# dmytroleonenko/gym-narde

Hardware: AMD Instinct MI355X
Metric: env steps/sec at batch=65536, 1 MI355X (+ legal-move bit-exact vs CPU) (higher is better)
Workload: dtype u32

## Files before the change

__graft_entry__.py:

```python
import os
import subprocess
import sys

ROOT = os.path.dirname(os.path.abspath(__file__))
PKG_DIR = os.path.join(ROOT, "gym-narde_amd")
CSRC = os.path.join(PKG_DIR, "csrc")
LIB = os.path.join(PKG_DIR, "gym_narde", "libnarde.so")
HOSTCHECK = os.path.join(ROOT, "tests", "hostcheck")

HIPCC = os.environ.get("HIPCC", "/opt/rocm/bin/hipcc")
HIP_FLAGS = ["-O3", "-std=c++17", "--offload-arch=gfx950", "-fPIC", "-shared", "-Wall"]


def _paths():
    for p in (PKG_DIR, os.path.join(ROOT, "oracle")):
        if p not in sys.path:
            sys.path.insert(0, p)


def _run(cmd):
    print("+", " ".join(cmd), flush=True)
    subprocess.check_call(cmd)


def build():
    srcs = [os.path.join(CSRC, "narde.hip"), os.path.join(CSRC, "dqn_learner.hip")]
    _run([HIPCC, *HIP_FLAGS, "-o", LIB, *srcs])
    _run(["make", "-s", "-C", os.path.join(ROOT, "oracle")])
    os.makedirs(os.path.join(HOSTCHECK, "build"), exist_ok=True)
    _run([HIPCC, "-O2", "-std=c++17", "-fPIC", "-shared", "-x", "c++", "-D__HIP_PLATFORM_AMD__",
          "-I/opt/rocm/include", "-o", os.path.join(HOSTCHECK, "build", "libhostcheck.so"),
          os.path.join(HOSTCHECK, "hostcheck.cpp")])
    _run([HIPCC, "-O2", "-std=c++17", "-fPIC", "-shared", "-x", "c++", "-D__HIP_PLATFORM_AMD__",
          "-I/opt/rocm/include", "-o", os.path.join(HOSTCHECK, "build", "libhostcheck_afterstates.so"),
          os.path.join(HOSTCHECK, "hostcheck_afterstates.cpp")])
    _run([HIPCC, "-O2", "-std=c++17", "-fPIC", "-shared", "-x", "c++", "-D__HIP_PLATFORM_AMD__",
          "-I/opt/rocm/include", "-o", os.path.join(HOSTCHECK, "build", "libhostcheck_turn_afterstates.so"),
          os.path.join(HOSTCHECK, "hostcheck_turn_afterstates.cpp")])
    _run([HIPCC, "-O2", "-std=c++17", "-fPIC", "-shared", "-x", "c++", "-D__HIP_PLATFORM_AMD__",
          "-I/opt/rocm/include", "-o", os.path.join(HOSTCHECK, "build", "libhostcheck_value.so"),
          os.path.join(HOSTCHECK, "hostcheck_value.cpp")])
    _run([HIPCC, "-O2", "-std=c++17", "-fPIC", "-shared", "-x", "c++", "-D__HIP_PLATFORM_AMD__",
          "-I/opt/rocm/include", "-o", os.path.join(HOSTCHECK, "build", "libhostcheck_td.so"),
          os.path.join(HOSTCHECK, "hostcheck_td.cpp")])
    _run([HIPCC, "-O2", "-std=c++17", "-fPIC", "-shared", "-x", "c++", "-D__HIP_PLATFORM_AMD__",
          "-I/opt/rocm/include", "-o", os.path.join(HOSTCHECK, "build", "libhostcheck_lookahead.so"),
          os.path.join(HOSTCHECK, "hostcheck_lookahead.cpp")])
    _run([HIPCC, "-O2", "-std=c++17", "-fPIC", "-shared", "-x", "c++", "-D__HIP_PLATFORM_AMD__",
          "-I/opt/rocm/include", "-o", os.path.join(HOSTCHECK, "build", "libhostcheck_turn_lookahead.so"),
          os.path.join(HOSTCHECK, "hostcheck_turn_lookahead.cpp")])
    _run([HIPCC, "-O2", "-std=c++17", "-fPIC", "-shared", "-x", "c++", "-D__HIP_PLATFORM_AMD__",
          "-I/opt/rocm/include", "-o", os.path.join(HOSTCHECK, "build", "libhostcheck_value_rollout.so"),
          os.path.join(HOSTCHECK, "hostcheck_value_rollout.cpp")])
    _run([HIPCC, "-O2", "-std=c++17", "-fPIC", "-shared", "-x", "c++", "-D__HIP_PLATFORM_AMD__",
          "-I/opt/rocm/include", "-o", os.path.join(HOSTCHECK, "build", "libhostcheck_turn_value_rollout.so"),
          os.path.join(HOSTCHECK, "hostcheck_turn_value_rollout.cpp")])
    _paths()
    import gym_narde
    import gym_narde.envs
    import gym_narde.vector
    from gym_narde import _lib

    _lib.load()


def smoke():
    _paths()
    import numpy as np
    import torch

    import oracle as O
    from gym_narde.envs.narde import Narde
    from gym_narde.vector import VecNardeEnv

    assert torch.cuda.is_available(), "smoke() needs a GPU"
    n, plies, seed = 2048, 64, 20251015
    env = VecNardeEnv(n, device="cuda:0", seed=seed, env_id_offset=5, max_episode_steps=1000)
    ref = O.SelfPlay(n, seed=seed, env0=5)
    ref.reset(0)
    rec = ref.run(plies)
    for p in range(plies):
        obs, rew, term, trunc, info = env.step()
        torch.cuda.synchronize()
        assert np.array_equal(obs.cpu().numpy(), rec["obs"][p].astype(np.int32)), f"obs ply {p}"
        assert np.array_equal(rew.cpu().numpy(), rec["reward"][p].astype(np.int32)), f"reward ply {p}"
        assert np.array_equal(term.cpu().numpy(), rec["terminated"][p]), f"terminated ply {p}"
        assert np.array_equal(info["actions"].cpu().numpy(), rec["action"][p]), f"actions ply {p}"
        assert np.array_equal(info["legal"].cpu().numpy().view(np.uint64), rec["legal"][p]), f"legal ply {p}"
    st = env.get_state()
    assert np.array_equal(st["board"].cpu().numpy(), ref.board)
    g = Narde()
    assert g.get_valid_moves([5, 3], 1) == [(23, 18)]
    assert g.get_valid_moves([6, 6], 1) == [(23, 17), (23, 17)]
    env.close()
    _smoke_turn_value_rollout(torch, VecNardeEnv, seed)
    print(f"smoke ok: {n} envs x {plies} plies bit-exact vs oracle; FULL4 value rollout = the composed loop")


def _smoke_turn_value_rollout(torch, VecNardeEnv, seed):
    from gym_narde.value_net import ValueMLP

    B, plies = 64, 3
    torch.manual_seed(seed)
    net = ValueMLP(80, "sigmoid", "sigmoid").to("cuda:0")
    one, loop = (VecNardeEnv(B, device="cuda:0", seed=seed, rules="full4") for _ in range(2))
    bufs = one.turn_value_rollout(plies, net)
    for k in range(plies):
        dice = loop.dice()
        aft, values = loop.scored_turn_afterstates(net, dice=dice)
# ... 21 lines not shown
```

gym-narde_amd/csrc/full4_wave.h:

```cpp
#pragma once

namespace {

__device__ __forceinline__ uint32_t rl(uint32_t v, int l) {
  return (uint32_t)__builtin_amdgcn_readlane((int)v, l);
}
__device__ void coop_run(const Side& s, uint32_t low, int a, int b, int hl, uint32_t m0, uint32_t m1,
                         int need, bool bf, int mode, int lane, uint32_t out[3]) {
  out[0] = out[1] = out[2] = 0u;
  uint64_t owners = __ballot((m0 | m1) != 0u);
  const int which = lane >> 5, p = lane & 31;
  while (owners) {
    const int ow = (int)__builtin_ctzll(owners);
    owners &= owners - 1ull;
    Side c;
    c.own.w[0] = rl(s.own.w[0], ow); c.own.w[1] = rl(s.own.w[1], ow); c.own.w[2] = rl(s.own.w[2], ow);
    c.O = rl(s.O, ow); c.S1o = rl(s.S1o, ow); c.P = rl(s.P, ow);
    c.off_own = rl(s.off_own, ow);
    c.opp.w[0] = c.opp.w[1] = c.opp.w[2] = 0u;
    c.S1p = 0u; c.off_opp = 0u; c.ft_own = 0u; c.ft_opp = 0u; c.black = 0u; c.elapsed = 0u; c.t = 0u;
    const uint32_t lw = rl(low, ow), om0 = rl(m0, ow), om1 = rl(m1, ow);
    const int pa = (int)rl((uint32_t)a, ow), pb = (int)rl((uint32_t)b, ow);
    const int thl = (int)rl((uint32_t)hl, ow), tneed = (int)rl((uint32_t)need, ow);
    const bool tbf = rl(bf ? 1u : 0u, ow) != 0u;
// ... 219 lines not shown
    c.O = rl(s.O, ow); c.S1o = rl(s.S1o, ow); c.P = rl(s.P, ow);
    c.off_own = rl(s.off_own, ow);
    c.opp.w[0] = c.opp.w[1] = c.opp.w[2] = 0u;
    c.S1p = 0u; c.off_opp = 0u; c.ft_own = 0u; c.ft_opp = 0u; c.black = 0u; c.elapsed = 0u; c.t = 0u;
    const uint32_t ofw = rl(fw, ow), om = rl(m0, ow), ow0 = rl(w0, ow);
    const int od = (int)rl((uint32_t)d, ow), ohl = (int)rl((uint32_t)hl, ow);
    const int nsrc = __builtin_popcount(om);
    const int r = lane >> 3, k = lane & 7;
    const bool hs = r < nsrc;
    const int s0 = select_bit(om, hs ? r : 0);
    Side ca = c;
    apply_die_if(ca, s0, od, hs);
    const int hla = ohl - ((hs && s0 == 23) ? 1 : 0);
    uint32_t L1 = die_candidates_sl(ca.O, ca.P, od);
    L1 &= ~block_reject_w(ca.O, ca.S1o, ofw, L1, od);
    L1 &= hla <= 0 ? ~HEAD : ~0u;
    L1 = hs ? L1 : 0u;
    const int cnt = __builtin_popcount(L1);
    if (nsrc > 8 || __ballot(k == 0 && cnt > 8) != 0ull) continue;
    const bool hp = k < cnt;
    const int s1 = select_bit(L1, hp ? k : 0);
    Side cp = ca;
    apply_die_if(cp, s1, od, hp);
    const int hlp = hla - ((hp && s1 == 23) ? 1 : 0);
    int dep = f4_probe_w<2>(cp, ofw, od, hlp);
    const bool miss = hp && dep == 1;
    if (__ballot(miss) != 0ull) {
      if (miss) dep = f4_depth_w<2>(cp, ofw, od, hlp);
    }
    const uint64_t B0 = __ballot(k == 0 && cnt > 0), B1 = __ballot(hp && dep >= 1), B2 = __ballot(hp && dep >= 2);
    const bool src = lane < 24 && ((om >> lane) & 1u);
    const int rt = __builtin_popcount(om & ((1u << (lane & 31)) - 1u));
    const int sh = src ? 8 * rt : 0;
    const uint32_t a0 = (uint32_t)__ballot(src && ((B0 >> sh) & 1ull) != 0ull);
    const uint32_t a1 = (uint32_t)__ballot(src && ((B1 >> sh) & 0xFFull) != 0ull);
    const uint32_t a2 = (uint32_t)__ballot(src && ((B2 >> sh) & 0xFFull) != 0ull);
    const int M = a2 ? 4 : (a1 ? 3 : (a0 ? 2 : 1));
    const uint32_t Cs = a2 ? a2 : (a1 ? a1 : (a0 ? a0 : om));
    const int p0 = select_bit(Cs, (int)mulhi_u32(ow0, (uint32_t)__builtin_popcount(Cs)));
    const int r0p = __builtin_popcount(om & ((1u << p0) - 1u));
    const uint32_t Lp = rl(L1, 8 * r0p);
    const uint32_t G = (uint32_t)(((M >= 4 ? B2 : B1) >> (8 * r0p)) & 0xFFull);
    const bool inl = lane < 24 && ((Lp >> lane) & 1u);
    const int e = __builtin_popcount(Lp & ((1u << (lane & 31)) - 1u));
    const uint32_t cv = (uint32_t)__ballot(inl && ((G >> e) & 1u));
    r0[0] = lane == ow ? a0 : r0[0];
    r0[1] = lane == ow ? a1 : r0[1];
    r0[2] = lane == ow ? a2 : r0[2];
    c1 = lane == ow ? cv : c1;
    ok = lane == ow ? true : ok;
  }
}

__device__ __forceinline__ void ply_bound_turn_c0(Side& s, int dh, int dl, uint32_t bs, uint32_t fw,
                                                  const uint32_t w[4], bool flip_always, TurnOut& o, int lane,
                                                  const TurnC0& c) {
  uint32_t Lh = c.Lh, Ll = c.Ll, Ch = c.Ch, Cl = c.Cl;
  int M = c.M;
  const int hl0 = c.hl0;
  const bool dbl = dh == dl;
  const bool b2 = bs != 0u && !dbl, bd = bs != 0u && dbl;
  if (__ballot(b2) != 0ull) {
    if (b2) turn_c0_pair_bound_w(s, dh, dl, bs, fw, Lh, Ll, Ch, Cl, M);
  }
  bool srch = false, pairs = false;
  uint32_t c1p = 0u;
  if (__ballot(bd) != 0ull) {
    const uint32_t Lb = Lh & ~block_reject_w(s.O, s.S1o, bd ? fw : 0u, Lh, dh);
    const bool fast = bd && f4_safe_bound(s, dh, hl0, bs) >= 4;
    srch = bd && !fast && Lb != 0u;
    uint32_t r0[3];
    coop_pair_w(s, fw, dh, hl0, srch ? Lb : 0u, w[0], lane, r0, c1p, pairs);
    if (__ballot(srch && !pairs) != 0ull) {
      uint32_t rd[3];
      coop_depth_w(s, fw, dh, hl0, (srch && !pairs) ? Lb : 0u, 3, lane, rd);
      if (srch && !pairs) { r0[0] = rd[0]; r0[1] = rd[1]; r0[2] = rd[2]; }
    }
    const int Ms = r0[2] ? 4 : (r0[1] ? 3 : (r0[0] ? 2 : 1));
    const uint32_t Cs = r0[2] ? r0[2] : (r0[1] ? r0[1] : (r0[0] ? r0[0] : Lb));
    Ch = bd ? (fast ? Lb : (Lb ? Cs : 0u)) : Ch;
    M = bd ? (fast ? 4 : (Lb ? Ms : 0)) : M;
  }
  o.legal = (uint64_t)Ch | ((uint64_t)Cl << 24) | ((uint64_t)dh << 48) | ((uint64_t)dl << 52) |
            ((uint64_t)M << 56);
  const int nh = __builtin_popcount(Ch), n = nh + __builtin_popcount(Cl);
  const int idx = (int)mulhi_u32(w[0], (uint32_t)n);
  const bool hi = idx < nh;
  const int d0 = hi ? dh : dl;
  const int p0 = select_bit(hi ? Ch : Cl, hi ? idx : idx - nh);
  const bool go = M >= 1;
  apply_die_if(s, p0, d0, go);
  uint32_t pl0 = go ? (0xFFFF0000u | ((uint32_t)d0 << 8) | (uint32_t)p0) : 0xFFFFFFFFu, pl1 = 0xFFFFFFFFu;
  int hl = hl0 - ((go && p0 == 23) ? 1 : 0);
  const int d1 = dbl ? dh : (d0 == dh ? dl : dh);
  const bool anyb = __ballot(bs != 0u) != 0ull;
#pragma unroll
  for (int k = 1; k < 4; ++k) {
    const int dk = k == 1 ? d1 : dh;
    const bool act = k < M;
    uint32_t Lk = die_candidates_sl(s.O, s.P, dk);
    if (anyb) {
      const bool filt = bd || (k == 1 && b2);
      Lk &= ~block_reject_w(s.O, s.S1o, filt ? fw : 0u, Lk, dk);
    }
    Lk &= hl <= 0 ? ~HEAD : ~0u;
    const int need = M - k - 1;
    const bool byp = k == 1 && pairs && need > 0;
    Lk = (srch && act && byp) ? c1p : Lk;
    const bool chk = srch && act && need > 0 && !byp;
    if (__ballot(chk) != 0ull) {
      uint32_t rk[3];
      coop_depth_w(s, fw, dk, hl, chk ? Lk : 0u, need, lane, rk);
      Lk = chk ? (need >= 2 ? rk[1] : rk[0]) : Lk;
    }
    const uint32_t wk = k == 1 ? w[1] : (k == 2 ? w[2] : w[3]);
    const int p = select_bit(Lk, (int)mulhi_u32(wk, (uint32_t)__builtin_popcount(Lk)));
    apply_die_if(s, p, dk, act);
    const uint32_t v = ((uint32_t)dk << 8) | (uint32_t)p;
    if (k == 1) pl0 = act ? ((pl0 & 0xFFFFu) | (v << 16)) : pl0;
    if (k == 2) pl1 = act ? ((pl1 & 0xFFFF0000u) | v) : pl1;
    if (k == 3) pl1 = act ? ((pl1 & 0xFFFFu) | (v << 16)) : pl1;
    hl -= (act && p == 23) ? 1 : 0;
  }
  o.played = (uint64_t)pl0 | ((uint64_t)pl1 << 32);
  o.max_dice = M;
  o.term = s.off_own == 15u;
  o.reward = o.term ? (s.off_opp > 0u ? 1 : 2) : 0;
  if (flip_always) side_flip(s);
  else side_flip_if(s, !o.term);
}

__device__ __forceinline__ void ply_bound_turn(Side& s, int dh, int dl, uint32_t bs, uint32_t fw, const uint32_t w[4],
                                               bool flip_always, TurnOut& o, int lane) {
  TurnC0 c;
  turn_c0_free(s, dh, dl, c.Lh, c.Ll, c.Ch, c.Cl, c.M, c.hl0);
  ply_bound_turn_c0(s, dh, dl, bs, fw, w, flip_always, o, lane, c);
}

}
```

gym-narde_amd/csrc/kernels_rollout.h:

```cpp
#pragma once

namespace {

struct Outs {
  int32_t* __restrict__ obs;
  int32_t* __restrict__ reward;
  uint8_t* __restrict__ term;
  uint8_t* __restrict__ trunc;
  uint64_t* __restrict__ legal;
  int16_t* __restrict__ act_out;
  uint64_t* __restrict__ played;
  int64_t* __restrict__ totals;
};

struct StepArgs {
  Planes pl;
  int n;
  Rng g;
  int max_steps;
  int autoreset;
  const int16_t* __restrict__ actions;
  const int8_t* __restrict__ play;
  const uint8_t* __restrict__ dice;
  Outs out;
// ... 97 lines not shown

__device__ __forceinline__ void store_outs(const Outs& out, size_t ix, const Side& s,
                                           const TurnOut& o, int term, int trunc, int4* lds,
                                           bool wave_full) {
  (void)wave_full;
  store_common(out, ix, s, o.reward, term, trunc, lds, false);
  if (out.legal) st_nt(out.legal + ix, o.legal);
  if (out.played) st_nt(out.played + ix, o.played);
}

#define OBS_LDS_DECL                                   \
  __shared__ int4 obs_lds[kBlock * 6];                 \
  int4* const wave_lds = obs_lds + (threadIdx.x & ~63) * 6;

__device__ __forceinline__ void ply_draw_cached(const Rng& g, uint32_t t, uint32_t i, uint32_t R[4], bool first,
                                                uint32_t r[4]) {
  if (first || (t & 1u) == 0u) ply_block(t, g.env0 + i, g.k0, g.k1, R);
  ply_words_of(R, t, g.dice_mode, r);
}

__device__ __forceinline__ void ply(Side& s, int4& st, const Rng& g, uint32_t i,
                                    const int16_t* actions, const uint8_t* dice, int max_steps,
                                    bool autoreset, StepOut& o, int& term, int& trunc, uint32_t R[4],
                                    bool first) {
  uint32_t r[4];
  ply_draw_cached(g, s.t, i, R, first, r);
  int d0 = 0, d1 = 0, c1 = 0, c2 = 0;
  if (dice) { d0 = dice[2 * i]; d1 = dice[2 * i + 1]; }
  if (actions) { c1 = actions[2 * i]; c2 = actions[2 * i + 1]; }
  if (!dice && !actions && autoreset) env_ply_policy_sl(s, st, r, g.dice_mode, max_steps, o, term, trunc);
  else env_ply(s, st, r, dice != nullptr, d0, d1, g.dice_mode, actions == nullptr, c1, c2, max_steps,
               autoreset, o, term, trunc);
}

__device__ __forceinline__ void ply_draw_wave(const Rng& g, uint32_t t, uint32_t i, uint32_t R[4], int p, int par,
                                              uint32_t r[4]) {
  if (par >= 0) {
    if (p == 0 || ((par + p) & 1) == 0) ply_block(t, g.env0 + i, g.k0, g.k1, R);
  } else if (p == 0 || (t & 1u) == 0u) {
    ply_block(t, g.env0 + i, g.k0, g.k1, R);
  }
  ply_words_of(R, t, g.dice_mode, r);
}

__device__ __forceinline__ int wave_parity(bool valid, uint32_t t) {
  const uint64_t odd = __ballot(valid && (t & 1u)), vm = __ballot(valid);
  return odd == 0ull ? 0 : (odd == vm ? 1 : -1);
}

template <bool kFilt>
__device__ __forceinline__ void ply_free_turn(Side& s, int dh, int dl, uint32_t bs, uint32_t fw, const uint32_t w[4],
                                              bool flip_always, TurnOut& o, const TurnC0& c) {
  uint32_t Lh = c.Lh, Ll = c.Ll, Ch = c.Ch, Cl = c.Cl;
  int M = c.M;
  const bool b2 = kFilt && bs != 0u;
  if (kFilt && b2) turn_c0_pair_bound_w(s, dh, dl, bs, fw, Lh, Ll, Ch, Cl, M);
  turn_moves_sl(s, dh, dl, Ch, Cl, M, c.hl0, w, b2, fw, flip_always, o);
}

__device__ __forceinline__ void ply_full_turn(Side& s, int4& st, int dh, int dl, uint32_t bs, uint32_t fw,
                                              const TurnC0& c, const uint32_t w[4], uint32_t rb, int max_steps,
                                              bool autoreset, TurnOut& o, int& term, int& trunc) {
  const uint32_t mover_black = s.black;
  if (__ballot(bs != 0u && dh == dl) == 0ull) {
    if (__ballot(bs != 0u) == 0ull) ply_free_turn<false>(s, dh, dl, bs, fw, w, autoreset, o, c);
    else ply_free_turn<true>(s, dh, dl, bs, fw, w, autoreset, o, c);
  } else {
    ply_bound_turn_c0(s, dh, dl, bs, fw, w, autoreset, o, (int)(threadIdx.x & 63), c);
  }
  if (autoreset) ply_close_sl_b(s, st, o.term, o.reward, mover_black, rb, max_steps, term, trunc);
  else ply_close(s, st, o.term, o.reward, mover_black, 0u, max_steps, false, term, trunc);
}

__device__ __forceinline__ void ply_full_dice(Side& s, int4& st, int dh, int dl, const uint32_t w[4], uint32_t rb,
                                              int max_steps, bool autoreset, TurnOut& o, int& term, int& trunc) {
  const uint32_t low = block_lowmask(s.P);
  uint32_t fw;
  const uint32_t bs = turn_block_set_sl(s.O, s.S1o, s.P, low, dh, dl, fw);
  TurnC0 c;
  turn_c0_free(s, dh, dl, c.Lh, c.Ll, c.Ch, c.Cl, c.M, c.hl0);
  ply_full_turn(s, st, dh, dl, bs, fw, c, w, rb, max_steps, autoreset, o, term, trunc);
}

__device__ __forceinline__ uint32_t ply_dice_word(const uint32_t r[4], int dice_mode, uint32_t w[4]) {
  int d0, d1;
  dice_from(r[0], dice_mode, d0, d1);
  const int dh = d0 > d1 ? d0 : d1, dl = d0 > d1 ? d1 : d0;
  turn_words(r, w);
  return (uint32_t)dh | ((uint32_t)dl << 4) | (reset_black(r[3]) << 8);
}

__device__ __forceinline__ void ply_full_words(Side& s, int4& st, const uint32_t r[4], int dice_mode,
                                               int max_steps, bool autoreset, TurnOut& o, int& term,
                                               int& trunc) {
  uint32_t w[4];
  const uint32_t dw = ply_dice_word(r, dice_mode, w);
  ply_full_dice(s, st, (int)(dw & 15u), (int)((dw >> 4) & 15u), w, autoreset ? dw >> 8 : 0u, max_steps, autoreset,
                o, term, trunc);
}

__device__ __forceinline__ void ply_policy_full(Side& s, int4& st, const Rng& g, uint32_t i, int max_steps,
                                                bool autoreset, TurnOut& o, int& term, int& trunc,
                                                uint32_t R[4], int p, int par) {
  uint32_t r[4];
  ply_draw_wave(g, s.t, i, R, p, par, r);
  ply_full_words(s, st, r, g.dice_mode, max_steps, autoreset, o, term, trunc);
}

__device__ __forceinline__ void ply(Side& s, int4& st, const Rng& g, uint32_t i, bool valid,
                                    const int8_t* play, const uint8_t* dice, int max_steps,
                                    bool autoreset, TurnOut& o, int& term, int& trunc, uint32_t R[4],
                                    bool first) {
  if (!play && !dice) {
    ply_policy_full(s, st, g, i, max_steps, autoreset, o, term, trunc, R, 0, 0);
    return;
  }
  uint32_t r[4];
  ply_draw_cached(g, s.t, i, R, first, r);
  int d0 = 1, d1 = 2;
  if (dice && valid) { d0 = dice[2 * i]; d1 = dice[2 * i + 1]; }
  const uint64_t pw = (play && valid) ? reinterpret_cast<const uint64_t*>(play)[i] : ~0ull;
  const int lane = (int)(threadIdx.x & 63);
  env_ply_full_with(s, st, r, g.env0 + i, g.k0, g.k1, dice != nullptr, d0, d1, g.dice_mode,
                    play != nullptr, pw, max_steps, autoreset, o, term, trunc,
                    [&](Side& s2, int a, int b, bool pl, uint64_t pw2, const uint32_t* w2, TurnOut& o2) {
                      coop_turn_full(s2, a, b, pl, pw2, w2, o2, lane);
                    });
}

__device__ __forceinline__ void add_stats(int4* __restrict__ stats, int i, const int4& st) {
  if (st.x) {
    int4 cur = stats[i];
    cur.x += st.x; cur.y += st.y; cur.z += st.z;
// ... 402 lines not shown
```

gym-narde_amd/csrc/narde_rules.h:

```cpp
#pragma once
#include <hip/hip_runtime.h>
#include <math.h>
#include <stdint.h>

#define NARDE_FN __host__ __device__ __forceinline__

namespace narde {

constexpr uint32_t MASK24 = 0xFFFFFFu;
constexpr int OFF = 24;

struct Nib {
  uint32_t w[3];
};

NARDE_FN uint32_t funnel16(uint32_t hi, uint32_t lo) { return (lo >> 16) | (hi << 16); }

NARDE_FN uint32_t nib_word(const Nib& b, int p) {
  const uint32_t w0 = b.w[0], w1 = b.w[1], w2 = b.w[2];
  const int k = p >> 3;
  return (k == 0 ? w0 : 0u) | (k == 1 ? w1 : 0u) | (k == 2 ? w2 : 0u);
}
NARDE_FN uint32_t nib_get(const Nib& b, int p) { return (nib_word(b, p) >> (4 * (p & 7))) & 15u; }
NARDE_FN void nib_add(Nib& b, int p, uint32_t delta ) {
// ... 1136 lines not shown
  return L & (e1 | e2 | e3);
}

NARDE_FN bool f4_bearoff_fixed_sl(const Side& s, int rem) {
  uint32_t x = s.own.w[0] & 0xFFFFFFu;
  x = (x & 0x0F0F0Fu) + ((x >> 4) & 0x0F0F0Fu);
  const uint32_t home = ((x * 0x010101u) >> 16) & 0xFFu;
  return ((s.O >> 6) == 0u) | ((int)(15u - s.off_own - home) >= rem);
}

NARDE_FN int f4_open_moves_sl(const Side& s, int d, int hl, int T) {
  const uint32_t O = s.O, fr = ~s.P & MASK24;
  const uint32_t r0 = (1u << d) - 1u;
  const uint32_t r1 = ((r0 & fr) << d) & MASK24;
  const uint32_t r2 = ((r1 & fr) << d) & MASK24;
  const uint32_t r3 = ((r2 & fr) << d) & MASK24;
  const uint32_t R = (r0 | r1 | r2 | r3) & O;
  const uint32_t h1 = ((0x3Fu & fr) << d) & MASK24;
  const uint32_t h2 = ((h1 & fr) << d) & MASK24;
  const uint32_t h3 = ((h2 & fr) << d) & MASK24;
  const uint32_t X = O & ~0x3Fu;
  const int head = (int)nib_get(s.own, 23);
  const bool reach = (X & ~(h1 | h2 | h3)) == 0u && !((X & HEAD) && head > hl);
  uint32_t ge4;
  const uint32_t ge3 = nib_ge3_ge4(s.own, ge4);
  const uint32_t Rb = R & ~HEAD;
  const int B = __builtin_popcount(Rb) + __builtin_popcount(Rb & ~s.S1o) + __builtin_popcount(Rb & ge3) +
                __builtin_popcount(Rb & ge4) + ((R & HEAD) ? head : 0);
  const int t = T + (reach ? B : 0);
  return t < 4 ? t : 4;
}

NARDE_FN void turn_c0_free(const Side& s, int dh, int dl, uint32_t& Lh, uint32_t& Ll, uint32_t& Ch, uint32_t& Cl,
                           int& M, int& hl0) {
  const bool dbl = dh == dl;
  Lh = die_candidates_sl(s.O, s.P, dh);
  Ll = die_candidates_sl(s.O, s.P, dl) & msk(!dbl);
  const uint32_t kh = f4_keep_pair_bf_sl(s.O, s.S1o, s.P, dh, dl, Lh);
  const uint32_t kl = f4_keep_pair_bf_sl(s.O, s.S1o, s.P, dl, dh, Ll);
  hl0 = (dbl && s.ft_own && (dh == 3 || dh == 4 || dh == 6)) ? 2 : 1;
  const int T0 = f4_exact_moves(s, dh, hl0);
  const int Mo = f4_open_moves_sl(s, dh, hl0, T0);
  const int Mx = f4_bearoff_fixed_sl(s, 4) ? T0 : Mo;
  const bool pair = (kh | kl) != 0u;
  const bool two = !dbl && pair;
  Ch = (kh & msk(two)) | (Lh & msk(!two));
  Cl = (kl & msk(two)) | (Ll & msk(!dbl && !pair && Lh == 0u));
  const int M2 = two ? 2 : ((Lh | Ll) != 0u ? 1 : 0);
  M = dbl ? (Lh != 0u ? Mx : 0) : M2;
}

struct TurnC0 {
  uint32_t Lh, Ll, Ch, Cl;
  int M, hl0;
};

NARDE_FN void side_flip_if(Side& s, bool flip) {
  Side f = s;
  side_flip(f);
  s.own.w[0] = flip ? f.own.w[0] : s.own.w[0];
  s.own.w[1] = flip ? f.own.w[1] : s.own.w[1];
  s.own.w[2] = flip ? f.own.w[2] : s.own.w[2];
  s.opp.w[0] = flip ? f.opp.w[0] : s.opp.w[0];
  s.opp.w[1] = flip ? f.opp.w[1] : s.opp.w[1];
  s.opp.w[2] = flip ? f.opp.w[2] : s.opp.w[2];
  s.O = flip ? f.O : s.O;
  s.P = flip ? f.P : s.P;
  s.S1o = flip ? f.S1o : s.S1o;
  s.S1p = flip ? f.S1p : s.S1p;
  s.off_own = flip ? f.off_own : s.off_own;
  s.off_opp = flip ? f.off_opp : s.off_opp;
  s.ft_own = flip ? f.ft_own : s.ft_own;
  s.ft_opp = flip ? f.ft_opp : s.ft_opp;
  s.black = flip ? f.black : s.black;
}

NARDE_FN uint32_t block_reject_w(uint32_t O, uint32_t S1, uint32_t fw, uint32_t C, int d);
NARDE_FN void turn_moves_sl(Side& s, int dh, int dl, uint32_t Ch, uint32_t Cl, int M, int hl, const uint32_t w[4],
                            bool filt, uint32_t fw, bool flip_always, TurnOut& o) {
  const bool dbl = dh == dl;
  o.legal = (uint64_t)Ch | ((uint64_t)Cl << 24) | ((uint64_t)dh << 48) | ((uint64_t)dl << 52) |
            ((uint64_t)M << 56);
  const int nh = __builtin_popcount(Ch), n = nh + __builtin_popcount(Cl);
  const int idx = (int)mulhi_u32(w[0], (uint32_t)n);
  const bool hi = idx < nh;
  const int d0 = hi ? dh : dl;
  const int p0 = select_bit(hi ? Ch : Cl, hi ? idx : idx - nh);
  const bool go = M >= 1;
  apply_die_if(s, p0, d0, go);
  uint32_t pl0 = go ? (0xFFFF0000u | ((uint32_t)d0 << 8) | (uint32_t)p0) : 0xFFFFFFFFu, pl1 = 0xFFFFFFFFu;
  hl -= (go && p0 == 23) ? 1 : 0;
  const int d1 = dbl ? dh : (d0 == dh ? dl : dh);
#pragma unroll
  for (int k = 1; k < 4; ++k) {
    const int dk = k == 1 ? d1 : dh;
    const bool act = k < M;
    uint32_t Lk = die_candidates_sl(s.O, s.P, dk);
    if (k == 1 && filt) Lk &= ~block_reject_w(s.O, s.S1o, fw, Lk, dk);
    Lk &= hl <= 0 ? ~HEAD : ~0u;
    const uint32_t wk = k == 1 ? w[1] : (k == 2 ? w[2] : w[3]);
    const int p = select_bit(Lk, (int)mulhi_u32(wk, (uint32_t)__builtin_popcount(Lk)));
    apply_die_if(s, p, dk, act);
    const uint32_t v = ((uint32_t)dk << 8) | (uint32_t)p;
    if (k == 1) pl0 = act ? ((pl0 & 0xFFFFu) | (v << 16)) : pl0;
    if (k == 2) pl1 = act ? ((pl1 & 0xFFFF0000u) | v) : pl1;
    if (k == 3) pl1 = act ? ((pl1 & 0xFFFFu) | (v << 16)) : pl1;
    hl -= (act && p == 23) ? 1 : 0;
  }
  o.played = (uint64_t)pl0 | ((uint64_t)pl1 << 32);
  o.max_dice = M;
  o.term = s.off_own == 15u;
  o.reward = o.term ? (s.off_opp > 0u ? 1 : 2) : 0;
  if (flip_always) side_flip(s);
  else side_flip_if(s, !o.term);
}

NARDE_FN void turn_free_sl(Side& s, int dh, int dl, const uint32_t w[4], bool flip_always, TurnOut& o) {
  uint32_t Lh, Ll, Ch, Cl;
  int M, hl0;
  turn_c0_free(s, dh, dl, Lh, Ll, Ch, Cl, M, hl0);
  turn_moves_sl(s, dh, dl, Ch, Cl, M, hl0, w, false, 0u, flip_always, o);
}


NARDE_FN void die_filter2(uint32_t O, uint32_t S1, const Blocks& bl, uint32_t Ca, int a, uint32_t Cb, int b,
                          uint32_t& La, uint32_t& Lb) {
  const uint32_t hitA = bl.F ? MASK24 : (bl.Q << a);
  const uint32_t hitB = bl.F ? MASK24 : (bl.Q << b);
  La = Ca & ~(hitA & ~S1);
  Lb = Cb & ~(hitB & ~S1);
  uint32_t ma = Ca & hitA & S1, mb = Cb & hitB & S1;
  while (ma | mb) {
    const bool fa = ma != 0u;
    const uint32_t m = fa ? ma : mb;
    const int d = fa ? a : b;
    const int p = __builtin_ctz(m);
    const uint32_t bp = 1u << p;
    ma &= fa ? ~bp : ~0u;
    mb &= fa ? ~0u : ~bp;
    const uint32_t Op = (O & ~bp) | (p >= d ? (1u << (p - d)) : 0u);
    const uint32_t rej = (runs6(Op) & bl.low) ? bp : 0u;
    La &= fa ? ~rej : ~0u;
    Lb &= fa ? ~0u : ~rej;
  }
}

NARDE_FN void legal2_low_sl(const Side& s, int d0, int d1, uint32_t low, Legal& l) {
  const int dh = d0 > d1 ? d0 : d1, dl = d0 > d1 ? d1 : d0;
  const bool dbl = dh == dl;
  const Blocks bl = block_info_low(s.O, low);
  uint32_t Lh, Ll;
  die_filter2(s.O, s.S1o, bl, die_candidates_sl(s.O, s.P, dh), dh,
              die_candidates_sl(s.O, s.P, dl) & msk(!dbl), dl, Lh, Ll);
  Ll = dbl ? Lh : Ll;
  const bool two_heads = s.ft_own && dbl && (dh == 3 || dh == 4 || dh == 6);
  Ll &= ((Lh >> 23) != 0u && !two_heads) ? ~HEAD : ~0u;
  l.n = 2;
  l.d[0] = dh; l.d[1] = dl; l.d[2] = 0; l.d[3] = 0;
  l.L[0] = Lh; l.L[1] = Ll; l.L[2] = 0u; l.L[3] = 0u;
  l.count = __builtin_popcount(Lh) + __builtin_popcount(Ll);
}

NARDE_FN void env_step_policy_sl(Side& s, int d0, int d1, uint32_t r1, uint32_t r2, StepOut& o) {
  const uint32_t low = block_lowmask(s.P);
  legal2_low_sl(s, d0, d1, low, o.l1);
  const int n1 = o.l1.count;
  int f1, t1;
  legal2_entry(o.l1, (int)mulhi_u32(r1, (uint32_t)n1), f1, t1);
  const int code1 = n1 >= 2 ? encode_move(f1, t1) : 0;
  const bool quirk = n1 >= 2 && t1 == 0 && f1 <= 5;
  const uint32_t bf1 = 1u << f1;
  const bool listed_off = (((o.l1.L[0] & bf1) != 0u) & (f1 < o.l1.d[0])) | (((o.l1.L[1] & bf1) != 0u) & (f1 < o.l1.d[1]));
  t1 = quirk ? OFF : t1;
  const bool play1 = quirk ? listed_off : n1 >= 1;
// ... 121 lines not shown

NARDE_FN uint32_t block_reject_w1(uint32_t O, uint32_t S1, uint32_t W, uint32_t C, int d) {
  const uint32_t H = W & ~O;
  const uint32_t stay = C & ~(W & S1);
  const uint32_t one = (H & (H - 1u)) == 0u ? (H << d) : 0u;
  return H == 0u ? stay : (stay & one & MASK24);
}
NARDE_FN uint32_t block_reject_w(uint32_t O, uint32_t S1, uint32_t fw, uint32_t C, int d) {
  uint32_t rej = block_reject_w1(O, S1, (0x3Fu << (__builtin_ctz(fw | 0x80000000u) & 31)) & MASK24, C, d);
  rej &= msk(fw != 0u);
  for (uint32_t f = fw & (fw - 1u); f; f &= f - 1u) rej |= block_reject_w1(O, S1, 0x3Fu << __builtin_ctz(f), C, d);
  return rej;
}

NARDE_FN bool pair_child_ok_w(const Side& s, uint32_t fw, int p, int a, int b) {
  uint32_t O2, S2;
  child_masks(s, p, a, O2, S2);
  const uint32_t Cb = die_candidates_sl(O2, s.P, b) & (p == 23 ? ~HEAD : ~0u);
  return (Cb & ~block_reject_w(O2, S2, fw, Cb, b)) != 0u;
}

NARDE_FN void turn_c0_pair_bound_w(const Side& s, int dh, int dl, uint32_t hs, uint32_t fw, uint32_t& Lh,
                                   uint32_t& Ll, uint32_t& Ch, uint32_t& Cl, int& M) {
  const uint32_t Chc = die_candidates_sl(s.O, s.P, dh), Clc = die_candidates_sl(s.O, s.P, dl);
  uint32_t rh = 0u, rl = 0u;
  for (uint32_t f = fw; f; f &= f - 1u) {
    const uint32_t W = 0x3Fu << __builtin_ctz(f);
    const uint32_t H = W & ~s.O;
    const bool one = (H & (H - 1u)) == 0u;
    const uint32_t keep = ~(W & s.S1o);
    rh |= H == 0u ? (Chc & keep) : (Chc & keep & (one ? (H << dh) : 0u) & MASK24);
    rl |= H == 0u ? (Clc & keep) : (Clc & keep & (one ? (H << dl) : 0u) & MASK24);
  }
  Lh = Chc & ~rh;
  Ll = Clc & ~rl;
  uint32_t kh = f4_sure_pair(s.O, s.P, dl, Lh, hs), kl = f4_sure_pair(s.O, s.P, dh, Ll, hs);
  uint32_t mh = Lh & ~kh, ml = Ll & ~kl;
  while (mh | ml) {
    const bool hi = mh != 0u;
    const int p = __builtin_ctz(hi ? mh : ml);
    const uint32_t bp = 1u << p;
    mh &= hi ? ~bp : ~0u;
    ml &= hi ? ~0u : ~bp;
    const bool ok = pair_child_ok_w(s, fw, p, hi ? dh : dl, hi ? dl : dh);
    kh |= (hi && ok) ? bp : 0u;
    kl |= (!hi && ok) ? bp : 0u;
  }
  const bool pair = (kh | kl) != 0u;
  Ch = pair ? kh : Lh;
  Cl = pair ? kl : (Lh ? 0u : Ll);
  M = pair ? 2 : ((Lh | Ll) ? 1 : 0);
}

NARDE_FN int obs_point(const Side& s, int p) { return (int)nib_get(s.own, p) - (int)nib_get(s.opp, p); }

NARDE_FN float tes_value(uint4 a, uint4 b, int col) {
  const bool black = (b.z >> 10) & 1u;
  const float player = (col == 196) != black ? 1.0f : 0.0f;
  const int side = col >= 98 ? 1 : 0;
  const int cc = col - 98 * side;
  const float offv = (float)(side ? ((b.z >> 4) & 15u) : (b.z & 15u)) / 15.0f;
  const int pt = cc < 96 ? (cc >> 2) : 0;
  const uint32_t w0 = side ? a.z : a.x, w1 = side ? a.w : a.y, w2 = side ? b.y : b.x;
  const int k = pt >> 3;
  const uint32_t word = k == 0 ? w0 : (k == 1 ? w1 : w2);
  const uint32_t v = (word >> (4 * (pt & 7))) & 15u;
  const int j = cc & 3;
  const float thr = v >= (uint32_t)(j + 1) ? 1.0f : 0.0f;
  const float over = v >= 3u ? (float)(v - 3u) / 2.0f : 0.0f;
  const float board = j == 3 ? over : thr;
  const float pv = cc == 96 ? 0.0f : (cc == 97 ? offv : board);
  return col >= 196 ? player : pv;
}

constexpr int kValHiddenMax = 128;
constexpr int kValLanes = 16;
constexpr int kValRows = 64 / kValLanes;
constexpr int kValUnits = kValHiddenMax / kValLanes;
constexpr int kValRowFirst = 6;
constexpr int kValRowSlots = 10;
constexpr int kValRootEach = 4;
constexpr int kValRootBatch = kValRows * kValRootEach;
constexpr int kValRootSlots = 48;
constexpr int kValRootItems = 51;
constexpr int64_t kValLdMax = 1 << 20;

NARDE_FN float tes_point_value(uint32_t v, int j) {
  const float thr = v >= (uint32_t)(j + 1) ? 1.0f : 0.0f;
  const float over = v >= 3u ? (float)(v - 3u) / 2.0f : 0.0f;
  return j == 3 ? over : thr;
}
NARDE_FN float tes_off_value(uint32_t off) { return (float)off / 15.0f; }

NARDE_FN uint32_t f32_bits(float x) { return __builtin_bit_cast(uint32_t, x); }
NARDE_FN float bits_f32(uint32_t x) { return __builtin_bit_cast(float, x); }

template <typename F>
NARDE_FN int tes_delta_walk(const uint4& a0, const uint4& b0, const uint4& a1, const uint4& b1, F&& emit) {
  int n = 0;
  for (int side = 0; side < 2; ++side) {
    const Nib r0{{side ? a0.z : a0.x, side ? a0.w : a0.y, side ? b0.y : b0.x}};
    const Nib r1{{side ? a1.z : a1.x, side ? a1.w : a1.y, side ? b1.y : b1.x}};
    const Nib x{{r0.w[0] ^ r1.w[0], r0.w[1] ^ r1.w[1], r0.w[2] ^ r1.w[2]}};
    for (uint32_t m = nz_mask(x); m; m &= m - 1u) {
      const int p = __builtin_ctz(m);
      const uint32_t u = nib_get(r0, p), v = nib_get(r1, p);
// ... 564 lines not shown
```

Before: 52.02 billion.

## Derive doubles move count from played dice instead of exact max-move search

Replaces the upfront exact maximum-moves computation for doubles (f4_exact_moves / open-move / bear-off checks) with a cap of 4. The actual count now comes from how many dice get played in the sequential loop, which stops at the first die with no legal move. This removes the expensive exact-move search per turn in the free and bound paths. It relies on greedy play reaching the same move count as the exact maximum, which must hold for the legal-move output to stay bit-exact. The legal word is also packed as two 32-bit halves.

```diff
diff --git a/__graft_entry__.py b/__graft_entry__.py
--- a/__graft_entry__.py
+++ b/__graft_entry__.py
@@ -55,6 +55,9 @@
     _run([HIPCC, "-O2", "-std=c++17", "-fPIC", "-shared", "-x", "c++", "-D__HIP_PLATFORM_AMD__",
           "-I/opt/rocm/include", "-o", os.path.join(HOSTCHECK, "build", "libhostcheck_turn_value_rollout.so"),
           os.path.join(HOSTCHECK, "hostcheck_turn_value_rollout.cpp")])
+    _run([HIPCC, "-O2", "-std=c++17", "-fPIC", "-shared", "-x", "c++", "-D__HIP_PLATFORM_AMD__",
+          "-I/opt/rocm/include", "-o", os.path.join(HOSTCHECK, "build", "libhostcheck_full4_count.so"),
+          os.path.join(HOSTCHECK, "hostcheck_full4_count.cpp")])
     _paths()
     import gym_narde
     import gym_narde.envs
diff --git a/gym-narde_amd/csrc/full4_wave.h b/gym-narde_amd/csrc/full4_wave.h
--- a/gym-narde_amd/csrc/full4_wave.h
+++ b/gym-narde_amd/csrc/full4_wave.h
@@ -299,7 +299,7 @@
                                                   const uint32_t w[4], bool flip_always, TurnOut& o, int lane,
                                                   const TurnC0& c) {
   uint32_t Lh = c.Lh, Ll = c.Ll, Ch = c.Ch, Cl = c.Cl;
-  int M = c.M;
+  int M = c.cap;
   const int hl0 = c.hl0;
   const bool dbl = dh == dl;
   const bool b2 = bs != 0u && !dbl, bd = bs != 0u && dbl;
@@ -324,8 +324,6 @@
     Ch = bd ? (fast ? Lb : (Lb ? Cs : 0u)) : Ch;
     M = bd ? (fast ? 4 : (Lb ? Ms : 0)) : M;
   }
-  o.legal = (uint64_t)Ch | ((uint64_t)Cl << 24) | ((uint64_t)dh << 48) | ((uint64_t)dl << 52) |
-            ((uint64_t)M << 56);
   const int nh = __builtin_popcount(Ch), n = nh + __builtin_popcount(Cl);
   const int idx = (int)mulhi_u32(w[0], (uint32_t)n);
   const bool hi = idx < nh;
@@ -337,10 +335,12 @@
   int hl = hl0 - ((go && p0 == 23) ? 1 : 0);
   const int d1 = dbl ? dh : (d0 == dh ? dl : dh);
   const bool anyb = __ballot(bs != 0u) != 0ull;
+  bool prev = go;
+  uint32_t cnt = go ? 1u : 0u;
 #pragma unroll
   for (int k = 1; k < 4; ++k) {
     const int dk = k == 1 ? d1 : dh;
-    const bool act = k < M;
+    const bool pre = prev && k < M;
     uint32_t Lk = die_candidates_sl(s.O, s.P, dk);
     if (anyb) {
       const bool filt = bd || (k == 1 && b2);
@@ -349,13 +349,14 @@
     Lk &= hl <= 0 ? ~HEAD : ~0u;
     const int need = M - k - 1;
     const bool byp = k == 1 && pairs && need > 0;
-    Lk = (srch && act && byp) ? c1p : Lk;
-    const bool chk = srch && act && need > 0 && !byp;
+    Lk = (srch && pre && byp) ? c1p : Lk;
+    const bool chk = srch && pre && need > 0 && !byp;
     if (__ballot(chk) != 0ull) {
       uint32_t rk[3];
       coop_depth_w(s, fw, dk, hl, chk ? Lk : 0u, need, lane, rk);
       Lk = chk ? (need >= 2 ? rk[1] : rk[0]) : Lk;
     }
+    const bool act = pre && Lk != 0u;
     const uint32_t wk = k == 1 ? w[1] : (k == 2 ? w[2] : w[3]);
     const int p = select_bit(Lk, (int)mulhi_u32(wk, (uint32_t)__builtin_popcount(Lk)));
     apply_die_if(s, p, dk, act);
@@ -364,9 +365,15 @@
     if (k == 2) pl1 = act ? ((pl1 & 0xFFFF0000u) | v) : pl1;
     if (k == 3) pl1 = act ? ((pl1 & 0xFFFFu) | (v << 16)) : pl1;
     hl -= (act && p == 23) ? 1 : 0;
-  }
+    prev = act;
+    cnt += act ? 1u : 0u;
+  }
+  const uint32_t Mf = bd ? (uint32_t)M : cnt;
+  const uint32_t lg0 = Ch | (Cl << 24);
+  const uint32_t lg1 = (Cl >> 8) | ((uint32_t)dh << 16) | ((uint32_t)dl << 20) | (Mf << 24);
+  o.legal = (uint64_t)lg0 | ((uint64_t)lg1 << 32);
   o.played = (uint64_t)pl0 | ((uint64_t)pl1 << 32);
-  o.max_dice = M;
+  o.max_dice = (int)Mf;
   o.term = s.off_own == 15u;
   o.reward = o.term ? (s.off_opp > 0u ? 1 : 2) : 0;
   if (flip_always) side_flip(s);
@@ -376,7 +383,7 @@
 __device__ __forceinline__ void ply_bound_turn(Side& s, int dh, int dl, uint32_t bs, uint32_t fw, const uint32_t w[4],
                                                bool flip_always, TurnOut& o, int lane) {
   TurnC0 c;
-  turn_c0_free(s, dh, dl, c.Lh, c.Ll, c.Ch, c.Cl, c.M, c.hl0);
+  turn_c0_cap(s, dh, dl, c.Lh, c.Ll, c.Ch, c.Cl, c.cap, c.hl0);
   ply_bound_turn_c0(s, dh, dl, bs, fw, w, flip_always, o, lane, c);
 }
 
diff --git a/gym-narde_amd/csrc/kernels_rollout.h b/gym-narde_amd/csrc/kernels_rollout.h
--- a/gym-narde_amd/csrc/kernels_rollout.h
+++ b/gym-narde_amd/csrc/kernels_rollout.h
@@ -173,10 +173,10 @@
 __device__ __forceinline__ void ply_free_turn(Side& s, int dh, int dl, uint32_t bs, uint32_t fw, const uint32_t w[4],
                                               bool flip_always, TurnOut& o, const TurnC0& c) {
   uint32_t Lh = c.Lh, Ll = c.Ll, Ch = c.Ch, Cl = c.Cl;
-  int M = c.M;
+  int cap = c.cap;
   const bool b2 = kFilt && bs != 0u;
-  if (kFilt && b2) turn_c0_pair_bound_w(s, dh, dl, bs, fw, Lh, Ll, Ch, Cl, M);
-  turn_moves_sl(s, dh, dl, Ch, Cl, M, c.hl0, w, b2, fw, flip_always, o);
+  if (kFilt && b2) turn_c0_pair_bound_w(s, dh, dl, bs, fw, Lh, Ll, Ch, Cl, cap);
+  turn_moves_cnt(s, dh, dl, Ch, Cl, cap, c.hl0, w, b2, fw, flip_always, o);
 }
 
 __device__ __forceinline__ void ply_full_turn(Side& s, int4& st, int dh, int dl, uint32_t bs, uint32_t fw,
@@ -199,7 +199,7 @@
   uint32_t fw;
   const uint32_t bs = turn_block_set_sl(s.O, s.S1o, s.P, low, dh, dl, fw);
   TurnC0 c;
-  turn_c0_free(s, dh, dl, c.Lh, c.Ll, c.Ch, c.Cl, c.M, c.hl0);
+  turn_c0_cap(s, dh, dl, c.Lh, c.Ll, c.Ch, c.Cl, c.cap, c.hl0);
   ply_full_turn(s, st, dh, dl, bs, fw, c, w, rb, max_steps, autoreset, o, term, trunc);
 }
 
diff --git a/gym-narde_amd/csrc/narde_rules.h b/gym-narde_amd/csrc/narde_rules.h
--- a/gym-narde_amd/csrc/narde_rules.h
+++ b/gym-narde_amd/csrc/narde_rules.h
@@ -1212,7 +1212,7 @@
 
 struct TurnC0 {
   uint32_t Lh, Ll, Ch, Cl;
-  int M, hl0;
+  int cap, hl0;
 };
 
 NARDE_FN void side_flip_if(Side& s, bool flip) {
@@ -1280,6 +1280,66 @@
   int M, hl0;
   turn_c0_free(s, dh, dl, Lh, Ll, Ch, Cl, M, hl0);
   turn_moves_sl(s, dh, dl, Ch, Cl, M, hl0, w, false, 0u, flip_always, o);
+}
+
+
+NARDE_FN void turn_c0_cap(const Side& s, int dh, int dl, uint32_t& Lh, uint32_t& Ll, uint32_t& Ch, uint32_t& Cl,
+                          int& cap, int& hl0) {
+  const bool dbl = dh == dl;
+  Lh = die_candidates_sl(s.O, s.P, dh);
+  Ll = die_candidates_sl(s.O, s.P, dl) & msk(!dbl);
+  const uint32_t kh = f4_keep_pair_bf_sl(s.O, s.S1o, s.P, dh, dl, Lh);
+  const uint32_t kl = f4_keep_pair_bf_sl(s.O, s.S1o, s.P, dl, dh, Ll);
+  hl0 = (dbl && s.ft_own && (dh == 3 || dh == 4 || dh == 6)) ? 2 : 1;
+  const bool pair = (kh | kl) != 0u;
+  const bool two = !dbl && pair;
+  Ch = (kh & msk(two)) | (Lh & msk(!two));
+  Cl = (kl & msk(two)) | (Ll & msk(!dbl && !pair && Lh == 0u));
+  const int M2 = two ? 2 : ((Lh | Ll) != 0u ? 1 : 0);
+  cap = dbl ? (Lh != 0u ? 4 : 0) : M2;
+}
+
+NARDE_FN void turn_moves_cnt(Side& s, int dh, int dl, uint32_t Ch, uint32_t Cl, int cap, int hl, const uint32_t w[4],
+                             bool filt, uint32_t fw, bool flip_always, TurnOut& o) {
+  const bool dbl = dh == dl;
+  const int nh = __builtin_popcount(Ch), n = nh + __builtin_popcount(Cl);
+  const int idx = (int)mulhi_u32(w[0], (uint32_t)n);
+  const bool hi = idx < nh;
+  const int d0 = hi ? dh : dl;
+  const int p0 = select_bit(hi ? Ch : Cl, hi ? idx : idx - nh);
+  const bool go = cap >= 1;
+  apply_die_if(s, p0, d0, go);
+  uint32_t pl0 = go ? (0xFFFF0000u | ((uint32_t)d0 << 8) | (uint32_t)p0) : 0xFFFFFFFFu, pl1 = 0xFFFFFFFFu;
+  hl -= (go && p0 == 23) ? 1 : 0;
+  const int d1 = dbl ? dh : (d0 == dh ? dl : dh);
+  bool act = go;
+  uint32_t M = go ? 1u : 0u;
+#pragma unroll
+  for (int k = 1; k < 4; ++k) {
+    const int dk = k == 1 ? d1 : dh;
+    uint32_t Lk = die_candidates_sl(s.O, s.P, dk);
+    if (k == 1 && filt) Lk &= ~block_reject_w(s.O, s.S1o, fw, Lk, dk);
+    Lk &= hl <= 0 ? ~HEAD : ~0u;
+    act = act && k < cap && Lk != 0u;
+    const uint32_t wk = k == 1 ? w[1] : (k == 2 ? w[2] : w[3]);
+    const int p = select_bit(Lk, (int)mulhi_u32(wk, (uint32_t)__builtin_popcount(Lk)));
+    apply_die_if(s, p, dk, act);
+    const uint32_t v = ((uint32_t)dk << 8) | (uint32_t)p;
+    if (k == 1) pl0 = act ? ((pl0 & 0xFFFFu) | (v << 16)) : pl0;
+    if (k == 2) pl1 = act ? ((pl1 & 0xFFFF0000u) | v) : pl1;
+    if (k == 3) pl1 = act ? ((pl1 & 0xFFFFu) | (v << 16)) : pl1;
+    hl -= (act && p == 23) ? 1 : 0;
+    M += act ? 1u : 0u;
+  }
+  const uint32_t lg0 = Ch | (Cl << 24);
+  const uint32_t lg1 = (Cl >> 8) | ((uint32_t)dh << 16) | ((uint32_t)dl << 20) | (M << 24);
+  o.legal = (uint64_t)lg0 | ((uint64_t)lg1 << 32);
+  o.played = (uint64_t)pl0 | ((uint64_t)pl1 << 32);
+  o.max_dice = (int)M;
+  o.term = s.off_own == 15u;
+  o.reward = o.term ? (s.off_opp > 0u ? 1 : 2) : 0;
+  if (flip_always) side_flip(s);
+  else side_flip_if(s, !o.term);
 }
 
 
```

Result: slower. 51.03 billion (-1.9%).

## Cooperatively evaluate bound pair-child checks across wavefront lanes

Applied to the files above, without the earlier changes.

Replaces the per-lane serial loop over candidate pair children in the bound-turn path with a wave-cooperative scheme. Each owning lane's state is broadcast via readlane and its candidate points are checked in parallel across lanes, with results gathered by ballot. The bound list and sure-pair filters are also recomputed with branch-free mask helpers. This aims to cut divergence in the serial per-lane loop, at the cost of broadcast overhead for each owner lane and running the helper even on lanes without bound pieces.

```diff
diff --git a/__graft_entry__.py b/__graft_entry__.py
--- a/__graft_entry__.py
+++ b/__graft_entry__.py
@@ -55,6 +55,9 @@
     _run([HIPCC, "-O2", "-std=c++17", "-fPIC", "-shared", "-x", "c++", "-D__HIP_PLATFORM_AMD__",
           "-I/opt/rocm/include", "-o", os.path.join(HOSTCHECK, "build", "libhostcheck_turn_value_rollout.so"),
           os.path.join(HOSTCHECK, "hostcheck_turn_value_rollout.cpp")])
+    _run([HIPCC, "-O2", "-std=c++17", "-fPIC", "-shared", "-x", "c++", "-D__HIP_PLATFORM_AMD__",
+          "-I/opt/rocm/include", "-o", os.path.join(HOSTCHECK, "build", "libhostcheck_pair_coop.so"),
+          os.path.join(HOSTCHECK, "hostcheck_pair_coop.cpp")])
     _paths()
     import gym_narde
     import gym_narde.envs
diff --git a/gym-narde_amd/csrc/full4_wave.h b/gym-narde_amd/csrc/full4_wave.h
--- a/gym-narde_amd/csrc/full4_wave.h
+++ b/gym-narde_amd/csrc/full4_wave.h
@@ -295,6 +295,41 @@
   }
 }
 
+__device__ void coop_pair_child_w(const Side& s, uint32_t fw, int dh, int dl, uint32_t mh, uint32_t ml, int lane,
+                                  uint32_t& kh, uint32_t& kl) {
+  const uint32_t dd = (uint32_t)dh | ((uint32_t)dl << 4);
+  const int which = lane >> 5, t = lane & 31;
+  for (uint64_t owners = __ballot((mh | ml) != 0u); owners; owners &= owners - 1ull) {
+    const int ow = (int)__builtin_ctzll(owners);
+    Side c{};
+    c.own.w[0] = rl(s.own.w[0], ow); c.own.w[1] = rl(s.own.w[1], ow); c.own.w[2] = rl(s.own.w[2], ow);
+    c.O = rl(s.O, ow); c.S1o = rl(s.S1o, ow); c.P = rl(s.P, ow);
+    const uint32_t ofw = rl(fw, ow), odd = rl(dd, ow), omh = rl(mh, ow), oml = rl(ml, ow);
+    const int odh = (int)(odd & 15u), odl = (int)(odd >> 4);
+    const bool has = t < 24 && (((which ? oml : omh) >> t) & 1u);
+    const bool ok = pair_child_ok_w(c, ofw, has ? t : 0, which ? odl : odh, which ? odh : odl);
+    const uint64_t r = __ballot(has && ok);
+    kh |= lane == ow ? (uint32_t)r : 0u;
+    kl |= lane == ow ? (uint32_t)(r >> 32) : 0u;
+  }
+}
+
+__device__ __forceinline__ void turn_c0_pair_bound_coop(const Side& s, int dh, int dl, uint32_t hs, uint32_t fw,
+                                                        bool b2, int lane, uint32_t& Lh, uint32_t& Ll, uint32_t& Ch,
+                                                        uint32_t& Cl, int& M) {
+  uint32_t fh, fl;
+  pair_bound_lists_w(s.O, s.S1o, b2 ? fw : 0u, Lh, Ll, dh, dl, fh, fl);
+  uint32_t kh = f4_sure_pair_sl(Ll, dl, fh, hs), kl = f4_sure_pair_sl(Lh, dh, fl, hs);
+  const uint32_t mh = b2 ? fh & ~kh : 0u, ml = b2 ? fl & ~kl : 0u;
+  if (__ballot((mh | ml) != 0u) != 0ull) coop_pair_child_w(s, fw, dh, dl, mh, ml, lane, kh, kl);
+  const bool pair = (kh | kl) != 0u;
+  Lh = b2 ? fh : Lh;
+  Ll = b2 ? fl : Ll;
+  Ch = b2 ? (pair ? kh : fh) : Ch;
+  Cl = b2 ? (pair ? kl : (fh ? 0u : fl)) : Cl;
+  M = b2 ? (pair ? 2 : ((fh | fl) ? 1 : 0)) : M;
+}
+
 __device__ __forceinline__ void ply_bound_turn_c0(Side& s, int dh, int dl, uint32_t bs, uint32_t fw,
                                                   const uint32_t w[4], bool flip_always, TurnOut& o, int lane,
                                                   const TurnC0& c) {
@@ -303,9 +338,7 @@
   const int hl0 = c.hl0;
   const bool dbl = dh == dl;
   const bool b2 = bs != 0u && !dbl, bd = bs != 0u && dbl;
-  if (__ballot(b2) != 0ull) {
-    if (b2) turn_c0_pair_bound_w(s, dh, dl, bs, fw, Lh, Ll, Ch, Cl, M);
-  }
+  if (__ballot(b2) != 0ull) turn_c0_pair_bound_coop(s, dh, dl, bs, fw, b2, lane, Lh, Ll, Ch, Cl, M);
   bool srch = false, pairs = false;
   uint32_t c1p = 0u;
   if (__ballot(bd) != 0ull) {
diff --git a/gym-narde_amd/csrc/kernels_rollout.h b/gym-narde_amd/csrc/kernels_rollout.h
--- a/gym-narde_amd/csrc/kernels_rollout.h
+++ b/gym-narde_amd/csrc/kernels_rollout.h
@@ -175,7 +175,7 @@
   uint32_t Lh = c.Lh, Ll = c.Ll, Ch = c.Ch, Cl = c.Cl;
   int M = c.M;
   const bool b2 = kFilt && bs != 0u;
-  if (kFilt && b2) turn_c0_pair_bound_w(s, dh, dl, bs, fw, Lh, Ll, Ch, Cl, M);
+  if (kFilt) turn_c0_pair_bound_coop(s, dh, dl, bs, fw, b2, (int)(threadIdx.x & 63), Lh, Ll, Ch, Cl, M);
   turn_moves_sl(s, dh, dl, Ch, Cl, M, c.hl0, w, b2, fw, flip_always, o);
 }
 
diff --git a/gym-narde_amd/csrc/narde_rules.h b/gym-narde_amd/csrc/narde_rules.h
--- a/gym-narde_amd/csrc/narde_rules.h
+++ b/gym-narde_amd/csrc/narde_rules.h
@@ -1507,6 +1507,34 @@
   M = pair ? 2 : ((Lh | Ll) ? 1 : 0);
 }
 
+NARDE_FN void pair_reject_w1(uint32_t O, uint32_t S1, uint32_t W, uint32_t Chc, uint32_t Clc, int dh, int dl,
+                             uint32_t& rh, uint32_t& rl) {
+  const uint32_t H = W & ~O;
+  const uint32_t keep = ~(W & S1) & MASK24;
+  const uint32_t hole = (H & (H - 1u)) == 0u ? H : 0u;
+  const uint32_t full = msk(H == 0u);
+  rh |= Chc & keep & (full | (hole << dh));
+  rl |= Clc & keep & (full | (hole << dl));
+}
+NARDE_FN void pair_bound_lists_w(uint32_t O, uint32_t S1, uint32_t fw, uint32_t Chc, uint32_t Clc, int dh, int dl,
+                                 uint32_t& Lh, uint32_t& Ll) {
+  uint32_t rh = 0u, rl = 0u;
+  pair_reject_w1(O, S1, (0x3Fu << (__builtin_ctz(fw | 0x80000000u) & 31)) & MASK24, Chc, Clc, dh, dl, rh, rl);
+  const uint32_t any = msk(fw != 0u);
+  rh &= any;
+  rl &= any;
+  for (uint32_t f = fw & (fw - 1u); f; f &= f - 1u) pair_reject_w1(O, S1, 0x3Fu << __builtin_ctz(f), Chc, Clc, dh, dl, rh, rl);
+  Lh = Chc & ~rh;
+  Ll = Clc & ~rl;
+}
+
+NARDE_FN uint32_t f4_sure_pair_sl(uint32_t Cb, int b, uint32_t La, uint32_t hs) {
+  const uint32_t safe = Cb & ~(hs << b);
+  const int c = __builtin_popcount(safe);
+  const uint32_t ok = msk(c >= 3) | (msk(c == 2) & ~(safe & (safe >> b))) | (msk(c == 1) & ~(safe | (safe >> b)));
+  return La & ok & msk(hs != ~0u);
+}
+
 NARDE_FN int obs_point(const Side& s, int p) { return (int)nib_get(s.own, p) - (int)nib_get(s.opp, p); }
 
 NARDE_FN float tes_value(uint4 a, uint4 b, int col) {
```

Result: no change. 52.01 billion before, 52.52 billion after (median of 5 runs) (+1.0%).
